# SingleRust/single-algebra

Measured on AMD Instinct MI355X. Metric: sparse_pca_fit_transform_algorithmic_throughput, higher is better.
Workload: dtype f32

## Files before the change

### single-algebra_amd/csrc/chol.hip

```cpp
#include "dense_common.h"

#include <algorithm>
#include <cmath>
#include <vector>

namespace sapca {
namespace k {

namespace {

__global__ void __launch_bounds__(256)
chol_inv_kernel(const double* __restrict__ G, int l, int ld, double* __restrict__ R, double* __restrict__ Rinv,
                int* __restrict__ info) {
  extern __shared__ double a[];
  const int st = l + 1;
  double* dinv = a + (size_t)l * st;
  __shared__ int bad;
  __shared__ double floor_s;
  const int tid = threadIdx.x;
  const int ti = tid >> 4, tj = tid & 15;
  if (tid == 0) bad = 0;
  for (int i = tid; i < l * l; i += blockDim.x) a[(i / l) * st + (i % l)] = G[(i / l) * ld + (i % l)];
  __syncthreads();
  if (tid == 0) {
    double scale = 0;
    for (int i = 0; i < l; ++i) scale = fmax(scale, fabs(a[i * st + i]));
    floor_s = scale * 1e-13 + 1e-300;
  }
  __syncthreads();
  for (int kk = 0; kk < l; ++kk) {
    if (tid == 0) {
      double v = a[kk * st + kk];
      if (!(v > floor_s)) { v = floor_s; bad += 1; }
      v = sqrt(v);
      a[kk * st + kk] = v;
      dinv[kk] = 1.0 / v;
    }
    __syncthreads();
    const double inv = dinv[kk];
    for (int j = kk + 1 + tid; j < l; j += blockDim.x) a[kk * st + j] *= inv;
    __syncthreads();
    for (int i = kk + 1 + ti; i < l; i += 16) {
      const double ri = a[kk * st + i];
      for (int j = kk + 1 + tj; j < l; j += 16)
        if (j >= i) a[i * st + j] -= ri * a[kk * st + j];
    }
    __syncthreads();
  }
  for (int j0 = 0; j0 < l; j0 += 64) {
    const int j = j0 + (tid >> 2), part = tid & 3;
    const bool live = j < l;
    const int jj = live ? j : 0;
    for (int i = l - 1; i >= 0; --i) {
      double s = 0;
      if (live && i < jj) {
        for (int t = i + 1 + part; t < jj; t += 4) s += a[i * st + t] * a[jj * st + t];
        if (part == 0) s += a[i * st + jj] * dinv[jj];
      }
      s += __shfl_xor(s, 1);
      s += __shfl_xor(s, 2);
      if (live && i < jj && part == 0) a[jj * st + i] = -s * dinv[i];
      __builtin_amdgcn_wave_barrier();
    }
  }
  __syncthreads();
  for (int i = tid; i < ld * ld; i += blockDim.x) {
    const int r = i / ld, c2 = i % ld;
    const bool in = r < l && c2 < l;
    R[i] = (in && c2 >= r) ? a[r * st + c2] : 0.0;
    Rinv[i] = !in ? 0.0 : (c2 > r ? a[c2 * st + r] : (c2 == r ? dinv[r] : 0.0));
  }
  if (tid == 0 && bad) atomicAdd(info, bad);
}

__device__ __forceinline__ double readlane_f64(double x, int lane) {
  const int lo = __builtin_amdgcn_readlane(__double2loint(x), lane);
  const int hi = __builtin_amdgcn_readlane(__double2hiint(x), lane);
  return __hiloint2double(hi, lo);
}

__device__ __forceinline__ void sqrt_rsqrt(double x, double& s, double& r) {
  const double y = __builtin_amdgcn_rsq(x);
  double g = x * y, h = 0.5 * y;
#pragma unroll
  for (int it = 0; it < 3; ++it) {
    const double e = fma(-h, g, 0.5);
    g = fma(g, e, g);
    h = fma(h, e, h);
  }
  g = fma(fma(-g, g, x), h, g);
  s = g;
  r = h + h;
}

__device__ __forceinline__ d4 block_mma(const double* pa, int sai, int sak, const double* pb, int sbk, int sbj, d4 acc,
                                        int lane) {
  const int i = lane & 15, g = lane >> 4;
  double a[4], b[4];
#pragma unroll
  for (int ks = 0; ks < 4; ++ks) {
    a[ks] = pa[i * sai + (4 * ks + g) * sak];
    b[ks] = pb[(4 * ks + g) * sbk + i * sbj];
  }
#pragma unroll
  for (int ks = 0; ks < 4; ++ks) acc = mfma_f64(a[ks], b[ks], acc);
  return acc;
}

constexpr int CHB = 16, CHN = 64, CHP = 65;
constexpr int kCholBlockedLds = (2 * CHN * CHP + 2 * CHN) * (int)sizeof(double);
#ifdef SAPCA_CHOL_TIMING
__device__ unsigned long long sapca_chol_stamps[32];
#define CHOL_STAMP(k) if (threadIdx.x == 0) sapca_chol_stamps[k] = __builtin_readcyclecounter();
#else
#define CHOL_STAMP(k)
#endif

__device__ __forceinline__ void invert_diag_block(const double* Lm, double* Xm, const double* dinvs, int c0, int lane) {
  const int r = lane & (CHB - 1);
  double a[CHB], x[CHB];
#pragma unroll
  for (int k = 0; k < CHB; ++k) a[k] = Lm[(c0 + r) * CHP + c0 + k];
  const double dmine = dinvs[c0 + r];
#pragma unroll
  for (int i = 0; i < CHB; ++i) {
    double s0 = 0.0, s1 = 0.0;
#pragma unroll
    for (int k = 0; k + 1 < i; k += 2) {
      s0 += readlane_f64(a[k], i) * x[k];
      s1 += readlane_f64(a[k + 1], i) * x[k + 1];
    }
    if (i & 1) s0 += readlane_f64(a[i - 1], i) * x[i - 1];
    const double di = readlane_f64(dmine, i);
    x[i] = i == r ? di : (i > r ? -(s0 + s1) * di : 0.0);
  }
  if (lane < CHB) {
#pragma unroll
    for (int i = 0; i < CHB; ++i) Xm[(c0 + i) * CHP + c0 + r] = x[i];
  }
}

template <bool STAMPS>
__device__ __forceinline__ void chol_inv_core(double* Lm, double* Xm, double* dinvs, int nb, double floor_s, int& bad) {
  const int t = threadIdx.x, wave = t >> 6, lane = t & 63;
  const int i16 = lane & 15, g4 = lane >> 4;
  for (int b = 0; b < nb; ++b) {
    const int c0 = b * CHB;
    if (wave == 0) {
      double a[CHB];
#pragma unroll
      for (int c = 0; c < CHB; ++c) a[c] = Lm[lane * CHP + c0 + c];
#pragma unroll
      for (int j = 0; j < CHB; ++j) {
        double piv = readlane_f64(a[j], c0 + j);
        if (!(piv > floor_s)) { piv = floor_s; bad += 1; }
        double d, dinv;
        sqrt_rsqrt(piv, d, dinv);
        a[j] = lane == c0 + j ? d : a[j] * dinv;
        if (lane == 0) dinvs[c0 + j] = dinv;
#pragma unroll
        for (int c = j + 1; c < CHB; ++c) a[c] -= a[j] * readlane_f64(a[j], c0 + c);
      }
#pragma unroll
      for (int c = 0; c < CHB; ++c)
        if (lane >= c0 + c) Lm[lane * CHP + c0 + c] = a[c];
    } else if (wave == 1 && b > 0) {
      invert_diag_block(Lm, Xm, dinvs, c0 - CHB, lane);
    }
    __syncthreads();
    if (STAMPS) { CHOL_STAMP(2 + 2 * b) }
    const int ntb = nb - b - 1, npairs = ntb * (ntb + 1) / 2;
    for (int p = wave; p < npairs; p += 4) {
      const int ii = p >= 3 ? 2 : (p >= 1 ? 1 : 0), jj = p - ii * (ii + 1) / 2;
      const int rI = (b + 1 + ii) * CHB, rJ = (b + 1 + jj) * CHB;
      d4 acc = d4{0, 0, 0, 0};
      acc = block_mma(Lm + rI * CHP + c0, CHP, 1, Lm + rJ * CHP + c0, 1, CHP, acc, lane);
#pragma unroll
      for (int reg = 0; reg < 4; ++reg) {
        const int row = rI + g4 + 4 * reg, col = rJ + i16;
        if (col <= row) Lm[row * CHP + col] -= acc[reg];
      }
    }
    __syncthreads();
    if (STAMPS) { CHOL_STAMP(3 + 2 * b) }
  }
  if (wave == 1) invert_diag_block(Lm, Xm, dinvs, (nb - 1) * CHB, lane);
  if (STAMPS) { CHOL_STAMP(10) }
  for (int bi = 1; bi < nb; ++bi) {
    if (bi == nb - 1) __syncthreads();
    const int bj = wave == 0 ? 0 : wave - 1;
    if (wave != 1 && bj < bi) {
      d4 tacc = d4{0, 0, 0, 0};
      for (int kb = bj; kb < bi; ++kb)
        tacc = block_mma(Lm + bi * CHB * CHP + kb * CHB, CHP, 1, Xm + kb * CHB * CHP + bj * CHB, CHP, 1, tacc, lane);
      d4 xacc = d4{0, 0, 0, 0};
      double a[4];
#pragma unroll
      for (int ks = 0; ks < 4; ++ks) a[ks] = Xm[(bi * CHB + i16) * CHP + bi * CHB + 4 * ks + g4];
#pragma unroll
      for (int ks = 0; ks < 4; ++ks) xacc = mfma_f64(a[ks], tacc[ks], xacc);
#pragma unroll
      for (int reg = 0; reg < 4; ++reg) Xm[(bi * CHB + g4 + 4 * reg) * CHP + bj * CHB + i16] = -xacc[reg];
      __builtin_amdgcn_fence(__ATOMIC_RELEASE, "wavefront");
      __builtin_amdgcn_wave_barrier();
    }
    if (STAMPS) { CHOL_STAMP(10 + bi) }
  }
  __syncthreads();
  if (STAMPS) {
    for (int bi = nb; bi < 4; ++bi) { CHOL_STAMP(10 + bi) }
  }
}

__global__ void __launch_bounds__(256)
chol_inv_blocked_kernel(const double* __restrict__ G, int l, int ld, double* __restrict__ R, double* __restrict__ Rinv,
                        int* __restrict__ info, const double* __restrict__ wsum, float* __restrict__ vec32, double* __restrict__ vec64) {
  extern __shared__ double cb_lds[];
  double* Lm = cb_lds;
  double* Xm = Lm + CHN * CHP;
  double* dinvs = Xm + CHN * CHP;
  double* ws = dinvs + CHN;
  if (wsum && threadIdx.x < CHN) ws[threadIdx.x] = (int)threadIdx.x < l ? wsum[threadIdx.x] : 0.0;
  const int t = threadIdx.x, lane = t & 63;
  const int nb = (l + CHB - 1) / CHB;
  CHOL_STAMP(0)
  double v[16];
#pragma unroll
  for (int u = 0; u < 16; ++u) {
    const int e = t + u * 256, i = e >> 6, c = e & 63;
    v[u] = (i < l && c <= i) ? G[(size_t)i * ld + c] : 0.0;
  }
  double dg = lane < l ? fabs(G[(size_t)lane * ld + lane]) : 0.0;
#pragma unroll
  for (int off = 32; off > 0; off >>= 1) dg = fmax(dg, __shfl_xor(dg, off));
  const double floor_s = dg * 1e-13 + 1e-300;
  const double pad = dg > 0.0 ? dg : 1.0;
#pragma unroll
  for (int u = 0; u < 16; ++u) {
    const int e = t + u * 256, i = e >> 6, c = e & 63;
    Lm[i * CHP + c] = (i >= l && i == c) ? pad : v[u];
    Xm[i * CHP + c] = 0.0;
  }
  __syncthreads();
  CHOL_STAMP(1)
  int bad = 0;
  chol_inv_core<true>(Lm, Xm, dinvs, nb, floor_s, bad);
  if (ld == CHN) {
#pragma unroll
    for (int u = 0; u < 16; ++u) {
      const int e = t + u * 256, r = e >> 6, c = e & 63;
      const bool in = r < l && c < l && c >= r;
      R[e] = in ? Lm[c * CHP + r] : 0.0;
      Rinv[e] = in ? Xm[c * CHP + r] : 0.0;
    }
  } else {
    for (int e = t; e < ld * ld; e += 256) {
      const int r = e / ld, c = e % ld;
      const bool in = r < l && c < l && c >= r;
      R[e] = in ? Lm[c * CHP + r] : 0.0;
      Rinv[e] = in ? Xm[c * CHP + r] : 0.0;
    }
  }
  CHOL_STAMP(14)
  if (wsum && t < ld) {
    double acc = 0;
    if (t < l)
      for (int i2 = 0; i2 <= t; ++i2) acc += Xm[t * CHP + i2] * ws[i2];
    if (vec32) vec32[t] = (float)acc;
    if (vec64) vec64[t] = acc;
  }
  if (t == 0 && bad) atomicAdd(info, bad);
}

__device__ __forceinline__ d4 mm_block(const double* pa, int sai, int sak, const double* pb, int sbk, int sbj, int nk, int lane) {
  d4 acc = d4{0, 0, 0, 0};
  for (int kb = 0; kb < nk; ++kb) acc = block_mma(pa + kb * CHB * sak, sai, sak, pb + kb * CHB * sbk, sbk, sbj, acc, lane);
  return acc;
}

constexpr int kChol128Lds = (4 * CHN * CHP + CHN) * (int)sizeof(double);

__global__ void __launch_bounds__(256)
chol_inv_blocked128_kernel(const double* __restrict__ G, int l, double* __restrict__ R, double* __restrict__ Rinv,
                           int* __restrict__ info) {
  constexpr int LD = 128;
  extern __shared__ double cb_lds[];
  double* B0 = cb_lds;
  double* B1 = B0 + CHN * CHP;
  double* B2 = B1 + CHN * CHP;
  double* B3 = B2 + CHN * CHP;
  double* dinvs = B3 + CHN * CHP;
  const int t = threadIdx.x, wave = t >> 6, lane = t & 63;
  const int i16 = lane & 15, g4 = lane >> 4;
  const int l2 = l - CHN, nb2 = (l2 + CHB - 1) / CHB;
  double dg = fabs(G[(size_t)lane * LD + lane]);
  if (lane + CHN < l) dg = fmax(dg, fabs(G[(size_t)(lane + CHN) * LD + lane + CHN]));
#pragma unroll
  for (int off = 32; off > 0; off >>= 1) dg = fmax(dg, __shfl_xor(dg, off));
  const double floor_s = dg * 1e-13 + 1e-300;
  const double pad = dg > 0.0 ? dg : 1.0;
  int bad = 0;
  {
    double v[16], w[16];
#pragma unroll
    for (int u = 0; u < 16; ++u) {
      const int e = t + u * 256, i = e >> 6, c = e & 63;
      v[u] = c <= i ? G[(size_t)i * LD + c] : 0.0;
      w[u] = i < l2 ? G[(size_t)(CHN + i) * LD + c] : 0.0;
    }
#pragma unroll
    for (int u = 0; u < 16; ++u) {
      const int e = t + u * 256, i = e >> 6, c = e & 63;
      B0[i * CHP + c] = v[u];
      B1[i * CHP + c] = 0.0;
      B2[i * CHP + c] = w[u];
    }
  }
  __syncthreads();
  chol_inv_core<false>(B0, B1, dinvs, 4, floor_s, bad);
#pragma unroll
  for (int u = 0; u < 16; ++u) {
    const int e = t + u * 256, r = e >> 6, c = e & 63;
    const bool in = c >= r;
    R[(size_t)r * LD + c] = in ? B0[c * CHP + r] : 0.0;
    Rinv[(size_t)r * LD + c] = in ? B1[c * CHP + r] : 0.0;
    R[(size_t)(CHN + r) * LD + c] = 0.0;
    Rinv[(size_t)(CHN + r) * LD + c] = 0.0;
  }
  for (int blk = wave; blk < 16; blk += 4) {
    const int I = blk >> 2, J = blk & 3;
    const d4 acc = mm_block(B2 + I * CHB * CHP, CHP, 1, B1 + J * CHB * CHP, 1, CHP, J + 1, lane);
#pragma unroll
    for (int reg = 0; reg < 4; ++reg) B3[(I * CHB + g4 + 4 * reg) * CHP + J * CHB + i16] = acc[reg];
  }
  __syncthreads();
  {
    double v[16];
#pragma unroll
    for (int u = 0; u < 16; ++u) {
      const int e = t + u * 256, i = e >> 6, c = e & 63;
      v[u] = (i < l2 && c <= i) ? G[(size_t)(CHN + i) * LD + CHN + c] : 0.0;
    }
#pragma unroll
    for (int u = 0; u < 16; ++u) {
      const int e = t + u * 256, i = e >> 6, c = e & 63;
      B0[i * CHP + c] = (i >= l2 && i == c) ? pad : v[u];
      B2[i * CHP + c] = 0.0;
      R[(size_t)i * LD + CHN + c] = c < l2 ? B3[c * CHP + i] : 0.0;
    }
  }
  __syncthreads();
  for (int p = wave; p < 10; p += 4) {
    const int I = p >= 6 ? 3 : (p >= 3 ? 2 : (p >= 1 ? 1 : 0)), J = p - I * (I + 1) / 2;
    const d4 acc = mm_block(B3 + I * CHB * CHP, CHP, 1, B3 + J * CHB * CHP, 1, CHP, 4, lane);
#pragma unroll
    for (int reg = 0; reg < 4; ++reg) {
      const int row = I * CHB + g4 + 4 * reg, col = J * CHB + i16;
      if (col <= row) B0[row * CHP + col] -= acc[reg];
    }
  }
  __syncthreads();
  chol_inv_core<false>(B0, B2, dinvs, nb2, floor_s, bad);
#pragma unroll
  for (int u = 0; u < 16; ++u) {
    const int e = t + u * 256, r = e >> 6, c = e & 63;
    const bool in = r < l2 && c < l2 && c >= r;
    R[(size_t)(CHN + r) * LD + CHN + c] = in ? B0[c * CHP + r] : 0.0;
    Rinv[(size_t)(CHN + r) * LD + CHN + c] = in ? B2[c * CHP + r] : 0.0;
  }
  __syncthreads();
  for (int blk = wave; blk < 16; blk += 4) {
    const int I = blk >> 2, J = blk & 3;
    const d4 acc = mm_block(B3 + I * CHB * CHP + J * CHB, CHP, 1, B1 + J * CHB * CHP + J * CHB, CHP, 1, 4 - J, lane);
#pragma unroll
    for (int reg = 0; reg < 4; ++reg) B0[(I * CHB + g4 + 4 * reg) * CHP + J * CHB + i16] = acc[reg];
  }
  __syncthreads();
  for (int blk = wave; blk < 16; blk += 4) {
    const int I = blk >> 2, J = blk & 3;
    const d4 acc = mm_block(B2 + I * CHB * CHP, CHP, 1, B0 + J * CHB, CHP, 1, I + 1, lane);
#pragma unroll
    for (int reg = 0; reg < 4; ++reg) B3[(I * CHB + g4 + 4 * reg) * CHP + J * CHB + i16] = -acc[reg];
  }
  __syncthreads();
#pragma unroll
  for (int u = 0; u < 16; ++u) {
    const int e = t + u * 256, r = e >> 6, c = e & 63;
    Rinv[(size_t)r * LD + CHN + c] = c < l2 ? B3[c * CHP + r] : 0.0;
  }
  if (t == 0 && bad) atomicAdd(info, bad);
}

template <typename T>
__global__ void rinv_tvec_kernel(const double* __restrict__ Rinv, int l, int ld, const double* __restrict__ wsum, T* __restrict__ vec) {
  const int j = blockIdx.x * blockDim.x + threadIdx.x;
  if (j >= ld) return;
  double s = 0;
  if (j < l)
    for (int i = 0; i <= j; ++i) s += Rinv[(size_t)i * ld + j] * wsum[i];
  vec[j] = (T)s;
}

}

static void chol_inv_host(const double* G, int l, int ld, double* R, double* Rinv, int* info, hipStream_t s) {
  std::vector<double> g((size_t)ld * ld);
  SAPCA_HIP(hipMemcpyAsync(g.data(), G, g.size() * sizeof(double), hipMemcpyDeviceToHost, s));
  SAPCA_HIP(hipStreamSynchronize(s));
  std::vector<double> a((size_t)l * l), r((size_t)ld * ld, 0.0), ri((size_t)ld * ld, 0.0), dinv((size_t)l);
  for (int i = 0; i < l; ++i)
    for (int j = 0; j < l; ++j) a[(size_t)i * l + j] = g[(size_t)i * ld + j];
  double scale = 0;
  for (int i = 0; i < l; ++i) scale = std::max(scale, std::fabs(a[(size_t)i * l + i]));
  const double floor_v = scale * 1e-13 + 1e-300;
  int bad = 0;
  for (int kk = 0; kk < l; ++kk) {
    double v = a[(size_t)kk * l + kk];
    if (!(v > floor_v)) { v = floor_v; ++bad; }
    v = std::sqrt(v);
    a[(size_t)kk * l + kk] = v;
    dinv[kk] = 1.0 / v;
    double* rk = &a[(size_t)kk * l];
    for (int j = kk + 1; j < l; ++j) rk[j] *= dinv[kk];
    for (int i = kk + 1; i < l; ++i) {
      const double rki = rk[i];
      double* ai = &a[(size_t)i * l];
      for (int j = i; j < l; ++j) ai[j] -= rki * rk[j];
    }
  }
  for (int i = l - 1; i >= 0; --i) {
    double* xi = &ri[(size_t)i * ld];
    xi[i] = dinv[i];
    for (int t = i + 1; t < l; ++t) {
      const double rit = a[(size_t)i * l + t];
      const double* xt = &ri[(size_t)t * ld];
      for (int j = t; j < l; ++j) xi[j] -= rit * xt[j];
    }
    for (int j = i + 1; j < l; ++j) xi[j] *= dinv[i];
  }
  for (int i = 0; i < l; ++i)
    for (int j = i; j < l; ++j) r[(size_t)i * ld + j] = a[(size_t)i * l + j];
  SAPCA_HIP(hipMemcpyAsync(R, r.data(), r.size() * sizeof(double), hipMemcpyHostToDevice, s));
  SAPCA_HIP(hipMemcpyAsync(Rinv, ri.data(), ri.size() * sizeof(double), hipMemcpyHostToDevice, s));
  if (bad) {
    int have = 0;
    SAPCA_HIP(hipMemcpyAsync(&have, info, sizeof(int), hipMemcpyDeviceToHost, s));
    SAPCA_HIP(hipStreamSynchronize(s));
    have += bad;
    SAPCA_HIP(hipMemcpyAsync(info, &have, sizeof(int), hipMemcpyHostToDevice, s));
  }
  SAPCA_HIP(hipStreamSynchronize(s));
}

enum class CholRoute { Blocked, Blocked128, General, Host };

static CholRoute chol_route(int l, int ld, bool general_only) {
  if (l > 128) return CholRoute::Host;
  if (general_only) return CholRoute::General;
  if (l <= 64 && ld >= l && ld <= 256) return CholRoute::Blocked;
  if (l > 64 && ld == 128) return CholRoute::Blocked128;
  return CholRoute::General;
}

void chol_inv(const double* G, int l, int ld, double* R, double* Rinv, int* info, hipStream_t s, const double* wsum, float* vec32, double* vec64) {
  static const bool general_only = dbg_env("SAPCA_CHOL_GENERAL") != nullptr;
  if (!vec32 && !vec64) wsum = nullptr;
  switch (chol_route(l, ld, general_only)) {
    case CholRoute::Blocked: {
      static LdsAttrState attr;
      ensure_dynamic_lds(reinterpret_cast<const void*>(&chol_inv_blocked_kernel), kCholBlockedLds, attr);
      hipLaunchKernelGGL(chol_inv_blocked_kernel, dim3(1), dim3(256), kCholBlockedLds, s, G, l, ld, R, Rinv, info, wsum, vec32, vec64);
      SAPCA_HIP(hipGetLastError());
      return;
    }
    case CholRoute::Blocked128: {
      static LdsAttrState attr;
      ensure_dynamic_lds(reinterpret_cast<const void*>(&chol_inv_blocked128_kernel), kChol128Lds, attr);
      hipLaunchKernelGGL(chol_inv_blocked128_kernel, dim3(1), dim3(256), kChol128Lds, s, G, l, R, Rinv, info);
      SAPCA_HIP(hipGetLastError());
      break;
    }
    case CholRoute::General: {
      const size_t lds = ((size_t)l * (l + 1) + l) * sizeof(double);
      static LdsAttrState attr;
      if (lds > 48 * 1024) ensure_dynamic_lds(reinterpret_cast<const void*>(&chol_inv_kernel), lds, attr);
      hipLaunchKernelGGL(chol_inv_kernel, dim3(1), dim3(256), lds, s, G, l, ld, R, Rinv, info);
      SAPCA_HIP(hipGetLastError());
      break;
    }
    case CholRoute::Host:
      chol_inv_host(G, l, ld, R, Rinv, info, s);
      break;
  }
  if (!wsum) return;
  if (vec32) hipLaunchKernelGGL((rinv_tvec_kernel<float>), dim3((ld + 63) / 64), dim3(64), 0, s, Rinv, l, ld, wsum, vec32);
  if (vec64) hipLaunchKernelGGL((rinv_tvec_kernel<double>), dim3((ld + 63) / 64), dim3(64), 0, s, Rinv, l, ld, wsum, vec64);
  SAPCA_HIP(hipGetLastError());
}

}
}
```

Baseline: 1392.

## Pipeline blocked Cholesky with lookahead panel factorization and overlapped triangular inverse

Restructures the blocked Cholesky-plus-inverse kernel into a lookahead schedule. The next panel's column update runs first so that wave 0 can factor it while the other waves finish the trailing updates and compute rows of the inverse interleaved with the factorization. This replaces the separate serial inverse sweep that ran afterwards. The panel factorization is also reordered so the next pivot's sqrt/rsqrt is computed early, shortening the dependency chain. The cost is more intricate cross-wave synchronization and a changed stamp layout.

After: 1392 (median of 3 runs). About the same (-0.0%).

```diff
diff --git a/single-algebra_amd/csrc/chol.hip b/single-algebra_amd/csrc/chol.hip
--- a/single-algebra_amd/csrc/chol.hip
+++ b/single-algebra_amd/csrc/chol.hip
@@ -140,76 +140,107 @@
   }
 }
 
+__device__ __forceinline__ void factor_block_column(double* Lm, double* dinvs, int c0, double floor_s, int& bad, int lane) {
+  double a[CHB];
+#pragma unroll
+  for (int c = 0; c < CHB; ++c) a[c] = Lm[lane * CHP + c0 + c];
+  double piv = readlane_f64(a[0], c0);
+  if (!(piv > floor_s)) { piv = floor_s; bad += 1; }
+  double d, dinv;
+  sqrt_rsqrt(piv, d, dinv);
+#pragma unroll
+  for (int j = 0; j < CHB; ++j) {
+    a[j] = lane == c0 + j ? d : a[j] * dinv;
+    if (lane == 0) dinvs[c0 + j] = dinv;
+    if (j + 1 < CHB) {
+      a[j + 1] -= a[j] * readlane_f64(a[j], c0 + j + 1);
+      piv = readlane_f64(a[j + 1], c0 + j + 1);
+      if (!(piv > floor_s)) { piv = floor_s; bad += 1; }
+      sqrt_rsqrt(piv, d, dinv);
+    }
+#pragma unroll
+    for (int c = j + 2; c < CHB; ++c) a[c] -= a[j] * readlane_f64(a[j], c0 + c);
+  }
+#pragma unroll
+  for (int c = 0; c < CHB; ++c)
+    if (lane >= c0 + c) Lm[lane * CHP + c0 + c] = a[c];
+}
+
+__device__ __forceinline__ void trailing_pair(double* Lm, int b, int I, int J, int lane) {
+  const int c0 = b * CHB, rI = I * CHB, rJ = J * CHB, i16 = lane & 15, g4 = lane >> 4;
+  d4 acc = d4{0, 0, 0, 0};
+  acc = block_mma(Lm + rI * CHP + c0, CHP, 1, Lm + rJ * CHP + c0, 1, CHP, acc, lane);
+#pragma unroll
+  for (int reg = 0; reg < 4; ++reg) {
+    const int row = rI + g4 + 4 * reg, col = rJ + i16;
+    if (col <= row) Lm[row * CHP + col] -= acc[reg];
+  }
+}
+
+__device__ __forceinline__ void xinv_finish_row(double* Xm, int bi, int bj, const d4& held, int lane) {
+  const int i16 = lane & 15, g4 = lane >> 4;
+  d4 xacc = d4{0, 0, 0, 0};
+  double a[4];
+#pragma unroll
+  for (int ks = 0; ks < 4; ++ks) a[ks] = Xm[(bi * CHB + i16) * CHP + bi * CHB + 4 * ks + g4];
+#pragma unroll
+  for (int ks = 0; ks < 4; ++ks) xacc = mfma_f64(a[ks], held[ks], xacc);
+#pragma unroll
+  for (int reg = 0; reg < 4; ++reg) Xm[(bi * CHB + g4 + 4 * reg) * CHP + bj * CHB + i16] = -xacc[reg];
+  __builtin_amdgcn_fence(__ATOMIC_RELEASE, "wavefront");
+  __builtin_amdgcn_wave_barrier();
+}
+
+__device__ __forceinline__ void xinv_round(const double* Lm, double* Xm, int r, int bj, d4& held, int lane) {
+  if (r - 2 > bj) xinv_finish_row(Xm, r - 2, bj, held, lane);
+  if (r - 1 > bj) {
+    const int bi = r - 1;
+    d4 tacc = d4{0, 0, 0, 0};
+    for (int kb = bj; kb < bi; ++kb)
+      tacc = block_mma(Lm + bi * CHB * CHP + kb * CHB, CHP, 1, Xm + kb * CHB * CHP + bj * CHB, CHP, 1, tacc, lane);
+    held = tacc;
+  }
+}
+
 template <bool STAMPS>
 __device__ __forceinline__ void chol_inv_core(double* Lm, double* Xm, double* dinvs, int nb, double floor_s, int& bad) {
   const int t = threadIdx.x, wave = t >> 6, lane = t & 63;
-  const int i16 = lane & 15, g4 = lane >> 4;
-  for (int b = 0; b < nb; ++b) {
-    const int c0 = b * CHB;
-    if (wave == 0) {
-      double a[CHB];
-#pragma unroll
-      for (int c = 0; c < CHB; ++c) a[c] = Lm[lane * CHP + c0 + c];
-#pragma unroll
-      for (int j = 0; j < CHB; ++j) {
-        double piv = readlane_f64(a[j], c0 + j);
-        if (!(piv > floor_s)) { piv = floor_s; bad += 1; }
-        double d, dinv;
-        sqrt_rsqrt(piv, d, dinv);
-        a[j] = lane == c0 + j ? d : a[j] * dinv;
-        if (lane == 0) dinvs[c0 + j] = dinv;
-#pragma unroll
-        for (int c = j + 1; c < CHB; ++c) a[c] -= a[j] * readlane_f64(a[j], c0 + c);
-      }
-#pragma unroll
-      for (int c = 0; c < CHB; ++c)
-        if (lane >= c0 + c) Lm[lane * CHP + c0 + c] = a[c];
-    } else if (wave == 1 && b > 0) {
-      invert_diag_block(Lm, Xm, dinvs, c0 - CHB, lane);
-    }
-    __syncthreads();
-    if (STAMPS) { CHOL_STAMP(2 + 2 * b) }
-    const int ntb = nb - b - 1, npairs = ntb * (ntb + 1) / 2;
-    for (int p = wave; p < npairs; p += 4) {
-      const int ii = p >= 3 ? 2 : (p >= 1 ? 1 : 0), jj = p - ii * (ii + 1) / 2;
-      const int rI = (b + 1 + ii) * CHB, rJ = (b + 1 + jj) * CHB;
-      d4 acc = d4{0, 0, 0, 0};
-      acc = block_mma(Lm + rI * CHP + c0, CHP, 1, Lm + rJ * CHP + c0, 1, CHP, acc, lane);
-#pragma unroll
-      for (int reg = 0; reg < 4; ++reg) {
-        const int row = rI + g4 + 4 * reg, col = rJ + i16;
-        if (col <= row) Lm[row * CHP + col] -= acc[reg];
-      }
-    }
+  const int xcol = wave == 0 ? 2 : wave - 2;
+  d4 held = d4{0, 0, 0, 0};
+  if (wave == 0) factor_block_column(Lm, dinvs, 0, floor_s, bad, lane);
+  __syncthreads();
+  if (STAMPS) { CHOL_STAMP(2) }
+  for (int c = 1; c < nb; ++c) {
+    const int b = c - 1;
+    if (wave < nb - c) trailing_pair(Lm, b, c + wave, c, lane);
     __syncthreads();
     if (STAMPS) { CHOL_STAMP(3 + 2 * b) }
+    if (wave == 0) {
+      factor_block_column(Lm, dinvs, c * CHB, floor_s, bad, lane);
+    } else {
+      const int ntb = nb - c - 1, npairs = ntb * (ntb + 1) / 2;
+      for (int p = wave - 1; p < npairs; p += 3) {
+        const int ii = p >= 3 ? 2 : (p >= 1 ? 1 : 0), jj = p - ii * (ii + 1) / 2;
+        trailing_pair(Lm, b, c + 1 + ii, c + 1 + jj, lane);
+      }
+      if (wave == 1) invert_diag_block(Lm, Xm, dinvs, b * CHB, lane);
+      else xinv_round(Lm, Xm, c, xcol, held, lane);
+    }
+    __syncthreads();
+    if (STAMPS) { CHOL_STAMP(2 + 2 * c) }
+  }
+  if (STAMPS) {
+    for (int s = 1 + 2 * nb; s < 10; ++s) { CHOL_STAMP(s) }
+    CHOL_STAMP(10)
   }
   if (wave == 1) invert_diag_block(Lm, Xm, dinvs, (nb - 1) * CHB, lane);
-  if (STAMPS) { CHOL_STAMP(10) }
-  for (int bi = 1; bi < nb; ++bi) {
-    if (bi == nb - 1) __syncthreads();
-    const int bj = wave == 0 ? 0 : wave - 1;
-    if (wave != 1 && bj < bi) {
-      d4 tacc = d4{0, 0, 0, 0};
-      for (int kb = bj; kb < bi; ++kb)
-        tacc = block_mma(Lm + bi * CHB * CHP + kb * CHB, CHP, 1, Xm + kb * CHB * CHP + bj * CHB, CHP, 1, tacc, lane);
-      d4 xacc = d4{0, 0, 0, 0};
-      double a[4];
-#pragma unroll
-      for (int ks = 0; ks < 4; ++ks) a[ks] = Xm[(bi * CHB + i16) * CHP + bi * CHB + 4 * ks + g4];
-#pragma unroll
-      for (int ks = 0; ks < 4; ++ks) xacc = mfma_f64(a[ks], tacc[ks], xacc);
-#pragma unroll
-      for (int reg = 0; reg < 4; ++reg) Xm[(bi * CHB + g4 + 4 * reg) * CHP + bj * CHB + i16] = -xacc[reg];
-      __builtin_amdgcn_fence(__ATOMIC_RELEASE, "wavefront");
-      __builtin_amdgcn_wave_barrier();
-    }
-    if (STAMPS) { CHOL_STAMP(10 + bi) }
-  }
-  __syncthreads();
-  if (STAMPS) {
-    for (int bi = nb; bi < 4; ++bi) { CHOL_STAMP(10 + bi) }
-  }
+  else xinv_round(Lm, Xm, nb, xcol, held, lane);
+  if (STAMPS) { CHOL_STAMP(11) }
+  __syncthreads();
+  if (STAMPS) { CHOL_STAMP(12) }
+  if (wave != 1 && nb - 1 > xcol) xinv_finish_row(Xm, nb - 1, xcol, held, lane);
+  __syncthreads();
+  if (STAMPS) { CHOL_STAMP(13) }
 }
 
 __global__ void __launch_bounds__(256)
```
